# snt-arg/visual_sgraphs

Hardware: AMD Instinct MI355X
Metric: frames/sec ORB extract+match @640x480, 1000 feats; bit-exact vs CPU (higher is better)
Workload: dtype u8; 1 GPU; C2: 640x480 gray, nFeatures=1000, 8 levels, scale 1.2, FAST 20/7, extract + brute-force Hamming best2 match vs previous frame; parallelism=frame-sharded x1

## Files before the change

include/vsg_orb.h:

```cpp
#ifndef VSG_ORB_H
#define VSG_ORB_H

#include <stddef.h>
#include <stdint.h>

#ifdef __cplusplus
extern "C" {
#endif

#define VSG_OK 0
#define VSG_ERR_EMPTY_IMAGE (-1)
#define VSG_ERR_CAPACITY (-2)
#define VSG_ERR_UNSUPPORTED (-3)
#define VSG_ERR_NO_DEVICE (-4)
#define VSG_ERR_HIP (-5)
#define VSG_ERR_INVALID (-6)
#define VSG_ERR_BUSY (-7)

typedef struct vsg_keypoint {
  float x, y, size, angle, response;
  int32_t octave, class_id;
} vsg_keypoint;

typedef struct vsg_orb vsg_orb;

const char *vsg_last_error(void);
int vsg_device_count(void);


int vsg_orb_create(int nfeatures, float scale_factor, int nlevels, int ini_th_fast, int min_th_fast, int device,
                   int max_batch, vsg_orb **out);
void vsg_orb_destroy(vsg_orb *h);

int vsg_orb_get_tables(const vsg_orb *h, float *scale, float *inv_scale, float *sigma2, float *inv_sigma2,
                       int *features_per_level, int *umax16);

int vsg_orb_set_blur_taps(vsg_orb *h, const uint16_t taps[7]);

int vsg_orb_set_pyramid_tiling(vsg_orb *h, int which);

int vsg_orb_capacity(vsg_orb *h, int rows, int cols);

int vsg_orb_extract(vsg_orb *h, const uint8_t *gray, int rows, int cols, int stride, int lap0, int lap1,
                    vsg_keypoint *kps, uint8_t *desc, int capacity, int *n);

int vsg_orb_extract_batch(vsg_orb *h, const uint8_t *gray, int nframes, size_t frame_stride, int rows, int cols,
                          int stride, int lap0, int lap1, vsg_keypoint *kps, uint8_t *desc, int capacity, int *n,
                          int *mono_index);

int vsg_orb_extract_batch_device(vsg_orb *h, const uint8_t *d_gray, int nframes, size_t frame_stride, int rows,
                                 int cols, int stride, int lap0, int lap1, vsg_keypoint *d_kps, uint8_t *d_desc,
                                 int *d_counts, int capacity, void *stream);

int vsg_orb_set_gray_coeffs(vsg_orb *h, const int coeffs[3], int shift);
// ... 292 lines not shown
```

include/vsg_orb_debug.h:

```cpp
#ifndef VSG_ORB_DEBUG_H
#define VSG_ORB_DEBUG_H
#include "vsg_orb.h"

#ifdef __cplusplus
extern "C" {
#endif

int vsg_debug_device_sort(int device, uint64_t *items, int n);

int vsg_debug_call_profile(float us[4]);

enum {
  VSG_OCT_BLUR_MEMBATCH = 1,
  VSG_OCT_BLUR_MEMBATCH_FUSED = 2,
  VSG_OCT_FEW_MEMBATCH = 3,
  VSG_OCT_FEW_MEMBATCH_FUSED = 4,
  VSG_OCT_STANDALONE = 5
};

typedef struct vsg_launch_forms {
  int latency_chain;
  int pyramid_tiling;
  int fast_cells_per_wg;
  int fast_tile_pitch;
  int cand_segmented;
  int fused_blur;
  int octree_kernel;
  int octree_hist_big;
  int octree_label_bytes;
  int octree_lead;
  int self_slots;
  int orient_mirror;
  int cus;
  int total_cells;
  int nframes;
} vsg_launch_forms;

int vsg_debug_last_launch_forms(vsg_orb *h, vsg_launch_forms *out);

#ifdef __cplusplus
}
#endif
#endif
```

visual_sgraphs_amd/csrc/vsg_kernels.h:

```cpp
#pragma once
#include <hip/hip_runtime.h>

#include "vsg_common.h"
#include "vsg_geometry.h"

namespace vsg {
struct OutMirror {
  KeyPointPOD *kps = nullptr;
  uint8_t *desc = nullptr;
  int *counts = nullptr;
  int capacity = 0;
};
void launch_stereo(hipStream_t s, const PyrView &pl, const PyrView &pr, float mb, float mbf, const float *scale,
                   const float *invScale, int nlevels, const KeyPointPOD *kpsL, const uint8_t *descL, int nL,
                   const KeyPointPOD *kpsR, const uint8_t *descR, int nR, float *uRight, float *depth, int *sadBest);
void launch_cvt_gray(hipStream_t s, const uint8_t *src, size_t sframe, int spitch, int channels, int rgb_order, int rows,
                     int cols, uint8_t *dst, size_t dframe, int dpitch, const int coeffs[3], int shift, int nframes);
void launch_zero(hipStream_t s, int *p, int n);
void launch_ingest(hipStream_t s, const uint8_t *src, size_t sframe, int spitch, uint8_t *dst, size_t dframe, int dpitch,
                   int rows, int cols, int nframes);
void launch_export(hipStream_t s, const KeyPointPOD *kps, const uint8_t *desc, const int *counts, int src_cap,
                   void *h_kps, void *h_desc, int *h_counts, int dst_cap, int nframes);
void launch_resize(hipStream_t s, uint8_t *pyr, const FrameGeom *d_fg, const Short4 *d_tab, const Src0 &s0,
                   const FrameGeom &fg, int level, int nframes);
void launch_pyramid(hipStream_t s, uint8_t *pyr, const FrameGeom *d_fg, const Short4 *d_tile_tab, const Src0 &s0,
                    const PyrTile *d_tiles, int ntiles, int ldsA, int ldsB, int tabMax, int nframes, int *cand_count);
struct FastForm {
  int cells_per_wg = 0, tile_pitch = 0;
};
struct OctreeForm {
  int kernel = 0;
  int hist_big = 0, label_bytes = 0, lead = 0;
};
FastForm launch_fast(hipStream_t s, const uint8_t *pyr, const FrameGeom *d_fg, const FastCellRec *d_recs, const Src0 &s0,
                     uint32_t *cand, int *cand_count, int *cell_count, const FrameGeom &fg, int maxVh, int maxVw, int maxArea,
                     int nframes, int cus);
OctreeForm launch_octree(hipStream_t s, const FrameGeom *d_fg, const uint32_t *cand, const int *cand_count,
                         const CellDesc *d_cells, const int *cell_count, uint32_t *cand2, uint16_t *node_of, uint32_t *sel,
                         int *sel_count, const FrameGeom &fg, int maxQuota, int maxCellsPerLevel, int nframes,
                         const uint8_t *blur_pyr = nullptr, uint8_t *blur_out = nullptr, const Src0 *blur_s0 = nullptr);
size_t octree_lds_bytes(const FrameGeom &fg, int maxQuota, int maxCellsPerLevel);
constexpr int kOctBlurWaves = 4;
void launch_debug_sort(hipStream_t s, uint64_t *d_items, int n);
void launch_blur(hipStream_t s, const uint8_t *pyr, uint8_t *blur, const FrameGeom *d_fg, const Src0 &s0,
                 const FrameGeom &fg, int nframes);
void launch_slots(hipStream_t s, const FrameGeom *d_fg, const uint32_t *sel, const int *sel_count, int *flags,
                  int4 *slots, FrameHeader *hdr, int lap0, int lap1, int nframes);
void launch_orient_desc(hipStream_t s, const uint8_t *pyr, const uint8_t *blur, const FrameGeom *d_fg, const Src0 &s0,
                        const uint32_t *sel, const int *sel_count, const int4 *slots, const FrameHeader *hdr,
                        const int8_t *pattern, KeyPointPOD *kps, uint8_t *desc, int *counts, int capacity,
                        const FrameGeom &fg, int nframes, const OutMirror &mir, bool self_slots);
void launch_border_copy(hipStream_t s, const uint8_t *img, int w, int h, int pitch, uint8_t *dst, int dpitch, int b);
}
```

visual_sgraphs_amd/csrc/vsg_kernels.hip:

```cpp
#include <hip/hip_runtime.h>
#include <stdint.h>
#include <stdlib.h>

#include "vsg_common.h"
#include "vsg_ctx.h"
#include "vsg_geometry.h"
#include "vsg_math.h"
#include "vsg_octree_core.h"
#include "vsg_kernels.h"
#include "../../include/vsg_orb_debug.h"

namespace vsg {

__device__ __forceinline__ const uint8_t *level_ptr(const FrameGeom *fg, const Src0 &s0, const uint8_t *pyr, int frame,
                                                    int level, int &pitch) {
  if (level == 0) {
    pitch = s0.pitch;
    return s0.base + (size_t)frame * s0.frame_stride;
  }
  pitch = fg->lv[level].pitch;
  return pyr + (size_t)frame * fg->pyr_frame_bytes + fg->lv[level].img_off;
}

struct BlockXY {
// ... 982 lines not shown
        const int cutA = K < nA ? (int)posA[K] : 0x7FFFFFFF, cutB = K >= 1 ? (int)posB[K - 1] : e;
        const int cut = cutA < cutB ? cutA : cutB;
        __threadfence_block();
        if (lane == 0) stk[3 * sp] = lo, stk[3 * sp + 1] = cut, stk[3 * sp + 2] = depth;
        sp++;
        lo = cut;
      }
      if (sp == 0) break;
      --sp;
      __threadfence_block();
      lo = stk[3 * sp], hi = stk[3 * sp + 1], depth = stk[3 * sp + 2];
    }
  }
};

constexpr int kOctRegPts = 8;

constexpr int kOctThreads = 256;
constexpr int kOctWaves = 5;

struct SegSrc {
  const uint32_t *level_cand;
  const int *prefix;
  const int *segoff;
  int ncells;
  __device__ int cell_of(int p) const {
    int lo = 0, hi = ncells;
    while (hi - lo > 1) {
      const int mid = (lo + hi) >> 1;
      if (prefix[mid] <= p) lo = mid; else hi = mid;
// ... 48 lines not shown

constexpr int kOctFewFrames = 8;
struct OctArgs {
  const FrameGeom *fg;
  const uint32_t *cand;
  const int *cand_count;
  const CellDesc *cells;
  const int *cell_count;
  uint32_t *cand2;
  uint16_t *node_of;
  uint32_t *sel;
  int *sel_count;
  int cap, prefix_off;
  int lab_off, lab_cap;
  int hist_big;
};

template <int kMemU>
__device__ __forceinline__ void octree_block(const OctArgs &a, int level, int frame, uint8_t *oct_lds, int *wtot,
                                             int *sort_stack) {
  const FrameGeom *__restrict__ fg = a.fg;
  const uint32_t *__restrict__ cand = a.cand;
  const int *__restrict__ cand_count = a.cand_count;
  const CellDesc *__restrict__ cells = a.cells;
  const int *__restrict__ cell_count = a.cell_count;
  uint32_t *__restrict__ cand2 = a.cand2;
  uint16_t *__restrict__ node_of = a.node_of;
  uint32_t *__restrict__ sel = a.sel;
  int *__restrict__ sel_count = a.sel_count;
  const int cap = a.cap, prefix_off = a.prefix_off;
// ... 66 lines not shown
      __syncthreads();
      if (npts <= a.lab_cap)
        n = octree::distribute<kMemU>(g, P, list, npts, (uint16_t *)(oct_lds + a.lab_off), W, out);
      else
        n = octree::distribute<kMemU>(g, P, list, npts, node_of + coff, W, out);
    }
  } else {
    int npts = cand_count[frame * kMaxLevels + level];
    if (npts > L.cand_cap) npts = L.cand_cap;
    n = npts <= kOctRegPts * kOctThreads ? octree::distribute_reg<kOctRegPts>(g, P, cand + coff, npts, W, out)
                                         : octree::distribute<kMemU>(g, P, cand + coff, npts, node_of + coff, W, out);
  }
  if (threadIdx.x == 0) sel_count[frame * kMaxLevels + level] = n;
}

constexpr int kOctMemBatch = 8, kOctMemBatchFused = 1;

__global__ __launch_bounds__(kOctThreads) __attribute__((amdgpu_waves_per_eu(kOctWaves, kOctWaves))) void k_octree(OctArgs a) {
  extern __shared__ __attribute__((aligned(16))) uint8_t oct_lds[];
  __shared__ int wtot[2 * kMaxWaves];
  __shared__ int sort_stack[kSortStackInts];
  octree_block<kOctMemBatch>(a, blockIdx.x, blockIdx.y, oct_lds, wtot, sort_stack);
}
template <int kMemU>
__global__ __launch_bounds__(kOctThreads) __attribute__((amdgpu_waves_per_eu(4, 4))) void k_octree_few(OctArgs a) {
  extern __shared__ __attribute__((aligned(16))) uint8_t oct_lds[];
  __shared__ int wtot[2 * kMaxWaves];
  __shared__ int sort_stack[kSortStackInts];
  octree_block<kMemU>(a, blockIdx.x, blockIdx.y, oct_lds, wtot, sort_stack);
}

__global__ __launch_bounds__(256) void k_debug_sort(uint64_t *items, int n) {
  extern __shared__ __attribute__((aligned(16))) uint8_t dbg_lds[];
  __shared__ int wtot[2 * kMaxWaves];
  __shared__ int sort_stack[kSortStackInts];
  introsort::item_t *buf = (introsort::item_t *)dbg_lds;
  uint16_t *posA = (uint16_t *)(buf + n), *posB = posA + n + 2;
  BlockGroup g;
  g.tid = threadIdx.x;
  g.nthreads = blockDim.x;
  g.wtot = wtot;
  g.stk = sort_stack;
  for (int i = g.tid; i < n; i += g.nthreads) buf[i] = items[i];
  __syncthreads();
// ... 163 lines not shown
        u32x4 line;
        line.x = q_hi ? r02 : c0, line.y = q_hi ? r13 : c1, line.z = q_hi ? c2 : r20, line.w = q_hi ? c3 : r31;
        *(u32x4 *)(dst + (uint32_t)(o >> 2) * tile_row_bytes) = line;
      }
    }
  }
}

__global__ __launch_bounds__(256) void k_blur(const uint8_t *__restrict__ pyr, uint8_t *__restrict__ blur,
                                              const FrameGeom *__restrict__ fg, Src0 s0) {
  blur_block<kBlurAheadAlone>(pyr, blur, fg, s0, frame_major_block());
}

template <int kMemU>
__device__ __forceinline__ void octree_blur_body(const OctArgs &a, const uint8_t *__restrict__ pyr, uint8_t *__restrict__ blur,
                                                 const Src0 &s0, int nlevels, int nframes, int lead, uint8_t *oct_lds, int *wtot,
                                                 int *sort_stack) {
  static_assert(kOctThreads == 256, "the blur body is written for 256-thread workgroups");
  BlockXY blk = frame_major_block();
  if (lead > 0) {
    if (blk.x >= nlevels) blk.y -= lead;
    if (blk.y < 0 || blk.y >= nframes) return;
  }
  if (blk.x < nlevels)
    octree_block<kMemU>(a, blk.x, blk.y, oct_lds, wtot, sort_stack);
  else
    blur_block<kBlurAheadFused>(pyr, blur, a.fg, s0, BlockXY{blk.x - nlevels, blk.y});
}
template <int kMemU>
__global__ __launch_bounds__(kOctThreads) __attribute__((amdgpu_waves_per_eu(kOctBlurWaves, kOctBlurWaves))) void k_octree_blur(
    OctArgs a, const uint8_t *__restrict__ pyr, uint8_t *__restrict__ blur, Src0 s0, int nlevels, int nframes, int lead) {
  extern __shared__ __attribute__((aligned(16))) uint8_t oct_lds[];
  __shared__ int wtot[2 * kMaxWaves];
  __shared__ int sort_stack[kSortStackInts];
  octree_blur_body<kMemU>(a, pyr, blur, s0, nlevels, nframes, lead, oct_lds, wtot, sort_stack);
}

__device__ __forceinline__ void slots_of_frame(const FrameGeom *__restrict__ fg, const uint32_t *__restrict__ sel,
                                               const int *__restrict__ sel_count, int *__restrict__ flags,
                                               int4 *__restrict__ slots, FrameHeader *__restrict__ hdr, int lap0, int lap1,
                                               int frame, int *wtot, int *lstart) {
  const int tid = threadIdx.x;
  if (tid == 0) {
    int s = 0;
    for (int l = 0; l < fg->nlevels; l++) {
      lstart[l] = s;
      s += min(sel_count[frame * kMaxLevels + l], fg->lv[l].sel_cap);
    }
    for (int l = fg->nlevels; l <= kMaxLevels; l++) lstart[l] = s;
  }
// ... 566 lines not shown
    return launch_fast_t<kFastThreads, 52, 52, 2 * (128 / kFastThreads)>(s, pyr, d_fg, d_recs, s0, cand, cand_count, cell_count, fg, maxVh, maxArea, nframes, cus);
  else if (maxVw <= 56)
    return launch_fast_t<kFastThreads, 68, 68, 3 * (128 / kFastThreads)>(s, pyr, d_fg, d_recs, s0, cand, cand_count, cell_count, fg, maxVh, maxArea, nframes, cus);
  else
    return launch_fast_t<kFastThreads, 84, 84, 4 * (128 / kFastThreads)>(s, pyr, d_fg, d_recs, s0, cand, cand_count, cell_count, fg, maxVh, maxArea, nframes, cus);
}
size_t octree_lds_bytes(const FrameGeom &fg, int maxQuota, int maxCellsPerLevel) {
  const int cap = octree::node_capacity(maxQuota);
  const size_t prefix_off = (octree::work_bytes(cap, false) + 15) & ~(size_t)15;
  return prefix_off + (fg.cand_segmented ? (2 * (size_t)maxCellsPerLevel + 1) * 4 : 0);
}

OctreeForm launch_octree(hipStream_t s, const FrameGeom *d_fg, const uint32_t *cand, const int *cand_count,
                         const CellDesc *d_cells, const int *cell_count, uint32_t *cand2, uint16_t *node_of, uint32_t *sel,
                         int *sel_count, const FrameGeom &fg, int maxQuota, int maxCellsPerLevel, int nframes,
                         const uint8_t *blur_pyr, uint8_t *blur_out, const Src0 *blur_s0) {
  const int cap = octree::node_capacity(maxQuota);
  const size_t prefix_bytes = fg.cand_segmented ? (2 * (size_t)maxCellsPerLevel + 1) * 4 : 0;
  const size_t share = 36 * 1024;
  const bool hist_big = ((octree::work_bytes(cap, true) + 15) & ~(size_t)15) + prefix_bytes <= share;
  const int prefix_off = (int)((octree::work_bytes(cap, hist_big) + 15) & ~(size_t)15);
  const size_t work_lds = (size_t)prefix_off + prefix_bytes;
  const size_t lab_off = (work_lds + 15) & ~(size_t)15;
  const size_t lab_bytes = work_lds <= 64 * 1024 && lab_off + 4096 <= share ? share - lab_off : 0;
  const size_t lds = lab_bytes ? lab_off + lab_bytes : work_lds;
  int dev = 0;
  hipGetDevice(&dev);
  const OctArgs a = {d_fg, cand, cand_count, d_cells, cell_count, cand2, node_of, sel, sel_count, cap, prefix_off,
                     (int)lab_off, (int)(lab_bytes / 2), hist_big ? 1 : 0};
  const bool few = nframes <= kOctFewFrames;
  OctreeForm form;
  form.hist_big = hist_big ? 1 : 0, form.label_bytes = (int)lab_bytes;
  if (blur_out) {
    constexpr int kLead = 64;
    const int lead = nframes >= 4 * kLead ? kLead : 0;
    form.lead = lead;
    const dim3 grid(fg.nlevels + fg.total_blur_blocks, nframes + lead);
    if (few && 5 * work_lds > 160 * 1024) {
      lds_limit_ensure(5, dev, (const void *)k_octree_blur<kOctMemBatch>, lds);
      hipLaunchKernelGGL(k_octree_blur<kOctMemBatch>, grid, dim3(kOctThreads), lds, s, a, blur_pyr, blur_out, *blur_s0,
                         fg.nlevels, nframes, lead);
      form.kernel = VSG_OCT_BLUR_MEMBATCH;
    } else {
      lds_limit_ensure(2, dev, (const void *)k_octree_blur<kOctMemBatchFused>, lds);
      hipLaunchKernelGGL(k_octree_blur<kOctMemBatchFused>, grid, dim3(kOctThreads), lds, s, a, blur_pyr, blur_out, *blur_s0,
                         fg.nlevels, nframes, lead);
      form.kernel = VSG_OCT_BLUR_MEMBATCH_FUSED;
    }
    return form;
  }
  dim3 grid(fg.nlevels, nframes), block(kOctThreads);
  if (few) {
    lds_limit_ensure(6, dev, (const void *)k_octree_few<kOctMemBatch>, lds);
    hipLaunchKernelGGL(k_octree_few<kOctMemBatch>, grid, block, lds, s, a);
    form.kernel = VSG_OCT_FEW_MEMBATCH;
    return form;
  }
  if (5 * work_lds <= 160 * 1024) {
    lds_limit_ensure(4, dev, (const void *)k_octree_few<kOctMemBatchFused>, lds);
    hipLaunchKernelGGL(k_octree_few<kOctMemBatchFused>, grid, block, lds, s, a);
    form.kernel = VSG_OCT_FEW_MEMBATCH_FUSED;
    return form;
  }
  lds_limit_ensure(1, dev, (const void *)k_octree, lds);
  hipLaunchKernelGGL(k_octree, grid, block, lds, s, a);
  form.kernel = VSG_OCT_STANDALONE;
// ... 39 lines not shown
```

visual_sgraphs_amd/csrc/vsg_orb.hip:

```cpp
#include <hip/hip_runtime.h>

#include <cstdio>
#include <cstdlib>
#include <algorithm>
#include <atomic>
#include <condition_variable>
#include <mutex>
#include <thread>
#include <chrono>
#include <cmath>
#include <cstring>
#include <map>
#include <string>
#include <utility>
#include <vector>

#include "../../include/vsg_orb.h"
#include "../../include/vsg_orb_debug.h"
#include "vsg_common.h"
#include "vsg_ctx.h"
#include "vsg_frame_int.h"
#include "vsg_geometry.h"
#include "vsg_kernels.h"

// ... 109 lines not shown
  int rows = 0, cols = 0;
  uint16_t taps[7] = {18, 34, 49, 55, 49, 34, 18};
  int gray_coeffs[3] = {4899, 9617, 1868};
  int gray_shift = 14;
  int last_frames = 0;
  vsg_launch_forms forms = {};
  bool have_forms = false;
  FrameGeom *d_fg = nullptr;
  Short4 *d_tab = nullptr;
  CellDesc *d_cells = nullptr;
  FastCellRec *d_fast = nullptr;
  int *d_cell_count = nullptr;
  uint32_t *d_cand2 = nullptr;
  int pyr_tiling = 0;
  int force_tiling = -1;
  vsg_post_chain_fn post_fn = nullptr;
  void *post_ctx = nullptr;
  int cus = 256;
  PyrTile *d_ptiles[kPyrTilings] = {};
  Short4 *d_ptab[kPyrTilings] = {};
  uint8_t *d_in = nullptr;
  int in_pitch = 0;
  Slot slot[kSlots];
  int next_ticket = 0;
  hipStream_t s_h2d = nullptr, s_d2h = nullptr;
  const KeyPointPOD *last_kps = nullptr;
  const uint8_t *last_desc = nullptr;
  const int *last_counts = nullptr;
  int last_cap = 0;
  hipEvent_t ev_last = nullptr;
// ... 151 lines not shown
    HIP_TRY(hipMalloc(&h->d_ptab[i], sizeof(Short4) * (PT.tab.size() + 1)));
    if (!PT.tab.empty())
      HIP_TRY(hipMemcpy(h->d_ptab[i], PT.tab.data(), sizeof(Short4) * PT.tab.size(), hipMemcpyHostToDevice));
  }
  HIP_TRY(hipMalloc(&h->d_pyr, B * fg.pyr_frame_bytes));
  HIP_TRY(hipMalloc(&h->d_blur, B * fg.blur_frame_bytes));
  HIP_TRY(hipMemset(h->d_pyr, 0, B * fg.pyr_frame_bytes));
  HIP_TRY(hipMemset(h->d_blur, 0, B * fg.blur_frame_bytes));
  HIP_TRY(hipMalloc(&h->d_cand, B * fg.cand_frame * sizeof(uint32_t)));
  HIP_TRY(hipMalloc(&h->d_cand2, B * fg.cand_frame * sizeof(uint32_t)));
  HIP_TRY(hipMalloc(&h->d_cell_count, B * fg.total_cells * sizeof(int)));
  HIP_TRY(hipMemset(h->d_cell_count, 0, B * fg.total_cells * sizeof(int)));
  HIP_TRY(hipStreamSynchronize(nullptr));
  HIP_TRY(hipMalloc(&h->d_nodeof, B * fg.cand_frame * sizeof(uint16_t)));
  HIP_TRY(hipMalloc(&h->d_sel, B * fg.sel_frame * sizeof(uint32_t)));
  HIP_TRY(hipMalloc(&h->d_counts2, 2 * B * kMaxLevels * sizeof(int)));
  HIP_TRY(hipMalloc(&h->d_flags, B * fg.out_cap * sizeof(int)));
  HIP_TRY(hipMalloc(&h->d_slots, B * fg.out_cap * sizeof(int4)));
  HIP_TRY(hipMalloc(&h->d_hdr, B * sizeof(FrameHeader)));
  h->in_pitch = (cols + 3) & ~3;
  HIP_TRY(hipMalloc(&h->d_in, B * (size_t)rows * h->in_pitch + 64));
  h->rows = rows;
  h->cols = cols;
  rc = ensure_slot(h, 0);
  if (rc != VSG_OK) return rc;
  h->pyr_tiling = 0;
  {
    const PyrTiling &P0 = h->G.pyr[0], &P1 = h->G.pyr[1];
    const int nf = h->max_batch;
    if (fg.nlevels > 1 && P0.ok && P1.ok && P0.lds_bytes() <= kPyrLdsLimit && P1.lds_bytes() <= 50 * 1024 &&
        (long long)P1.tiles.size() * nf >= 2048) {
// ... 39 lines not shown

static int enqueue_pipeline(vsg_orb *h, const Src0 &s0, int nf, int lap0, int lap1, KeyPointPOD *d_kps,
                            uint8_t *d_desc, int *d_counts, int capacity, hipStream_t s) {
  h->last_src0 = s0;
  const FrameGeom &fg = h->G.fg;
  const bool tm = h->timing;
  const bool tmf = !tm && h->timing_fast;
  if (tm || tmf) harvest_timing(h);
  hipStream_t sb = h->serialize ? s : kOwnBlurStream;
  uint8_t *pyr = h->d_pyr, *blur = h->d_blur;
  uint32_t *cand = h->d_cand, *sel = h->d_sel;
  uint16_t *nodeof = h->d_nodeof;
  int *cell_count = h->d_cell_count;
  int *cand_count = h->d_counts2;
  int *sel_count = h->d_counts2 + (size_t)h->max_batch * kMaxLevels;
  int *flags = h->d_flags;
  int4 *slots = h->d_slots;
  FrameHeader *hdr = h->d_hdr;
  vsg_launch_forms &rec = h->forms;
  rec = vsg_launch_forms();
  rec.cus = h->cus, rec.total_cells = fg.total_cells, rec.nframes = nf, rec.cand_segmented = fg.cand_segmented ? 1 : 0;
  h->have_forms = true;
  Range r_all("vsg_orb: enqueue stage chain");
  if (tm) HIP_TRY(hipEventRecord(h->ev[0], s));
  int ti = -1;
  if (fg.nlevels > 1) {
    const PyrTiling &P0 = h->G.pyr[0], &P1 = h->G.pyr[1];
    const PyrTiling &PS = h->G.pyr[kPyrTilingSmall];
    const int forced = h->force_tiling;
    if (forced == 3)
// ... 21 lines not shown
  if (tm) HIP_TRY(hipEventRecord(h->ev[1], s));
  if (tm || tmf) HIP_TRY(hipEventRecord(h->ev[8], s));
  const FastForm ff = launch_fast(s, pyr, h->d_fg, h->d_fast, s0, cand, cand_count, cell_count, fg, h->G.fastMaxVh,
                                  h->G.fastMaxVw, h->G.fastMaxArea, nf, h->cus);
  rec.fast_cells_per_wg = ff.cells_per_wg, rec.fast_tile_pitch = ff.tile_pitch;
  if (tm || tmf) HIP_TRY(hipEventRecord(h->ev[2], s));
  constexpr int kFusedLdsWorkgroups = 5;
  const bool lds_fits = kFusedLdsWorkgroups * octree_lds_bytes(fg, h->G.maxQuota, h->G.maxCellsPerLevel) <= 160 * 1024;
  const bool fused_blur = !tm && sb != s && (lds_fits || (h->one_stream && nf <= 8));
  const bool self_slots = !tm && (lap1 < kEdgeThreshold || lap0 > lap1);
  rec.fused_blur = fused_blur ? 1 : 0, rec.self_slots = self_slots ? 1 : 0;
  OctreeForm of;
  if (fused_blur) {
    Range r_tail("DistributeOctTree (+ blur workgroups) + slots + IC_Angle / rBRIEF");
    of = launch_octree(s, h->d_fg, cand, cand_count, h->d_cells, cell_count, h->d_cand2, nodeof, sel, sel_count, fg,
                       h->G.maxQuota, h->G.maxCellsPerLevel, nf, pyr, blur, &s0);
    if (!self_slots) launch_slots(s, h->d_fg, sel, sel_count, flags, slots, hdr, lap0, lap1, nf);
  } else {
    HIP_TRY(hipEventRecord(h->ev_pyr, s));
    if (sb == kOwnBlurStream) {
      const int rs = need_stream(h, &h->s_blur);
      if (rs != VSG_OK) return rs;
      sb = h->s_blur;
    }
    const bool octree_first = sb != s;
    if (octree_first) {
      if (tm) HIP_TRY(hipEventRecord(h->ev[10], s));
      of = launch_octree(s, h->d_fg, cand, cand_count, h->d_cells, cell_count, h->d_cand2, nodeof, sel, sel_count, fg,
                         h->G.maxQuota, h->G.maxCellsPerLevel, nf);
      if (tm) HIP_TRY(hipEventRecord(h->ev[3], s));
    }
    HIP_TRY(hipStreamWaitEvent(sb, h->ev_pyr, 0));
    if (tm) HIP_TRY(hipEventRecord(h->ev[6], sb));
    launch_blur(sb, pyr, blur, h->d_fg, s0, fg, nf);
    if (tm) HIP_TRY(hipEventRecord(h->ev[7], sb));
    HIP_TRY(hipEventRecord(h->ev_blur, sb));
    Range r_tail("DistributeOctTree + slots + IC_Angle / rBRIEF");
    if (!octree_first) {
      if (tm) HIP_TRY(hipEventRecord(h->ev[10], s));
      of = launch_octree(s, h->d_fg, cand, cand_count, h->d_cells, cell_count, h->d_cand2, nodeof, sel, sel_count, fg,
                         h->G.maxQuota, h->G.maxCellsPerLevel, nf);
      if (tm) HIP_TRY(hipEventRecord(h->ev[3], s));
    }
    if (!self_slots) launch_slots(s, h->d_fg, sel, sel_count, flags, slots, hdr, lap0, lap1, nf);
    if (tm) HIP_TRY(hipEventRecord(h->ev[4], s));
    HIP_TRY(hipStreamWaitEvent(s, h->ev_blur, 0));
    if (tm) HIP_TRY(hipEventRecord(h->ev[9], s));
  }
  rec.octree_kernel = of.kernel, rec.octree_hist_big = of.hist_big, rec.octree_label_bytes = of.label_bytes;
  rec.octree_lead = of.lead;
  rec.orient_mirror = h->mirror.kps ? 1 : 0;
  launch_orient_desc(s, pyr, blur, h->d_fg, s0, sel, sel_count, slots, hdr, h->d_pattern, d_kps, d_desc, d_counts,
                     capacity, fg, nf, h->mirror, self_slots);
  if (tm) HIP_TRY(hipEventRecord(h->ev[5], s));
  if (tm || tmf) h->ev_pending = true;
  HIP_TRY(hipGetLastError());
  h->last_frames = nf;
  h->last_kps = d_kps, h->last_desc = d_desc, h->last_counts = d_counts, h->last_cap = capacity;
  HIP_TRY(hipEventRecord(h->ev_last, s));
  h->have_last = true;
  return VSG_OK;
}

static int wait_last(vsg_orb *h) {
  if (h->have_last) HIP_TRY(hipEventSynchronize(h->ev_last));
// ... 232 lines not shown
  if (tsum > 257) return VSG_ERR_UNSUPPORTED;
  memcpy(h->taps, taps, sizeof(h->taps));
  if (h->rows) {
    for (int k = 0; k < 7; k++) h->G.fg.taps[k] = taps[k];
    HIP_TRY(hipSetDevice(h->device));
    int rc = quiesce(h);
    if (rc != VSG_OK) return rc;
    HIP_TRY(hipMemcpy(h->d_fg, &h->G.fg, sizeof(FrameGeom), hipMemcpyHostToDevice));
  }
  return VSG_OK;
}

int vsg_orb_set_pyramid_tiling(vsg_orb *h, int which) {
  if (!h || which < -1 || which > kPyrTilings) return VSG_ERR_INVALID;
  h->force_tiling = which;
  return VSG_OK;
}

int vsg_orb_capacity(vsg_orb *h, int rows, int cols) {
  if (!h) return VSG_ERR_INVALID;
  if (rows <= 0 || cols <= 0) return VSG_ERR_EMPTY_IMAGE;
  int rc = ensure_geometry(h, rows, cols);
  if (rc != VSG_OK) return rc;
  return h->G.fg.out_cap;
}

int vsg_orb_extract_batch_device(vsg_orb *h, const uint8_t *d_gray, int nframes, size_t frame_stride, int rows,
                                 int cols, int stride, int lap0, int lap1, vsg_keypoint *d_kps, uint8_t *d_desc,
                                 int *d_counts, int capacity, void *stream) {
  if (!h || !d_kps || !d_desc || !d_counts || nframes < 1 || nframes > h->max_batch) return VSG_ERR_INVALID;
// ... 679 lines not shown
  launch_debug_sort(c->stream, (uint64_t *)c->d_buf, n);
  HIP_TRY(hipGetLastError());
  HIP_TRY(hipMemcpyAsync(c->h_pin, c->d_buf, sizeof(uint64_t) * n, hipMemcpyDeviceToHost, c->stream));
  HIP_TRY(hipStreamSynchronize(c->stream));
  memcpy(items, c->h_pin, sizeof(uint64_t) * n);
  return VSG_OK;
}

int vsg_debug_last_launch_forms(vsg_orb *h, vsg_launch_forms *out) {
  if (!h || !out) return VSG_ERR_INVALID;
  if (!h->have_forms) {
    set_err("vsg_debug_last_launch_forms: the handle has not enqueued a batch yet");
    return VSG_ERR_INVALID;
  }
  *out = h->forms;
  return VSG_OK;
}

int vsg_orb_get_timing(vsg_orb *h, float *ms_out, int cap) {
  if (!h) return VSG_ERR_INVALID;
  harvest_timing(h);
  for (int i = 0; i < kStages && i < cap; i++) ms_out[i] = h->acc_n ? (float)(h->acc_ms[i] / h->acc_n) : 0.f;
  return kStages;
}

}
```

visual_sgraphs_amd/orb.py:

```python
import ctypes as C
from pathlib import Path

import numpy as np

import os

_PKG = Path(__file__).resolve().parent
LIB_PATH = Path(os.environ["VSG_LIB"]) if os.environ.get("VSG_LIB") else _PKG / "libvsg_orb.so"

KP_DTYPE = np.dtype([("x", "<f4"), ("y", "<f4"), ("size", "<f4"), ("angle", "<f4"), ("response", "<f4"),
                     ("octave", "<i4"), ("class_id", "<i4")])
assert KP_DTYPE.itemsize == 28

VSG_OK = 0
ERRORS = {-1: "VSG_ERR_EMPTY_IMAGE", -2: "VSG_ERR_CAPACITY", -3: "VSG_ERR_UNSUPPORTED", -4: "VSG_ERR_NO_DEVICE",
          -5: "VSG_ERR_HIP", -6: "VSG_ERR_INVALID", -7: "VSG_ERR_BUSY"}

_u8p = C.POINTER(C.c_uint8)
_i32p = C.POINTER(C.c_int32)
_u32p = C.POINTER(C.c_uint32)
_f32p = C.POINTER(C.c_float)
_u16p = C.POINTER(C.c_uint16)

EXPORTS = [
# ... 9 lines not shown
    "vsg_vocab_info", "vsg_bow_transform", "vsg_distinctive_descriptors", "vsg_debug_device_sort",
    "vsg_search_for_triangulation", "vsg_search_by_bow_kf_f_stereo",
    "vsg_thread_release", "vsg_thread_arena_growths", "vsg_debug_call_profile", "vsg_orb_time_stats", "vsg_host_register", "vsg_host_unregister", "vsg_host_alloc", "vsg_host_free", "vsg_orb_slots",
    "vsg_orb_submit_batch", "vsg_orb_wait", "vsg_orb_copy_pyramid", "vsg_frame_create", "vsg_frame_destroy",
    "vsg_frame_upload", "vsg_frame_from_extractor", "vsg_frame_size", "vsg_frame_copy_grid",
    "vsg_frame_features_in_area", "vsg_frame_search_by_projection", "vsg_frame_search_by_projection_last",
    "vsg_frame_search_by_projection_sim3", "vsg_frame_search_by_projection_kf", "vsg_frame_search_by_sim3",
    "vsg_frame_fuse", "vsg_frame_fuse_sim3", "vsg_fuse_decide", "vsg_frame_search_for_initialization",
    "vsg_frame_search_by_bow_kf_f", "vsg_frame_search_by_bow_kf_kf", "vsg_frame_bow_transform", "vsg_frame_stereo_bow_search",
    "vsg_frame_search_for_triangulation",
    "vsg_frame_stereo_matches",
    "vsg_shard_last_error", "vsg_shard_record_bytes", "vsg_shard_record_desc_offset", "vsg_shard_frame_owner",
    "vsg_shard_stream_owner", "vsg_shard_unique_id", "vsg_shard_create", "vsg_shard_destroy", "vsg_shard_all_gather",
    "vsg_shard_record", "vsg_shard_world", "vsg_shard_send_recv_boundary", "vsg_shard_boundary_record",
    "vsg_copy_d2d_async",
    "vsg_orb_set_pyramid_tiling", "vsg_shard_rank", "vsg_camera_image_bounds", "vsg_frame_from_extractor_undistort",
    "vsg_orb_extract_to_frame",
    "vsg_orb_extract_to_frame_rgbd", "vsg_depth_map_scale", "vsg_rgbd_depth_batch_device",
    "vsg_host_kind", "vsg_orb_set_direct_registered",
    "vsg_vocab_score", "vsg_kfdb_create", "vsg_kfdb_destroy", "vsg_kfdb_add", "vsg_kfdb_erase", "vsg_kfdb_clear",
    "vsg_kfdb_clear_map", "vsg_kfdb_set_map", "vsg_kfdb_set_covisibility", "vsg_kfdb_detect_relocalization_candidates",
    "vsg_kfdb_detect_n_best_candidates",
    "vsg_mappoints_create", "vsg_mappoints_destroy", "vsg_mappoints_capacity", "vsg_mappoints_update",
    "vsg_mappoints_read", "vsg_frame_is_in_frustum", "vsg_frame_search_local_points",
    "vsg_debug_last_launch_forms",
]

LAUNCH_FORM_FIELDS = ("latency_chain", "pyramid_tiling", "fast_cells_per_wg", "fast_tile_pitch", "cand_segmented",
                      "fused_blur", "octree_kernel", "octree_hist_big", "octree_label_bytes", "octree_lead", "self_slots",
                      "orient_mirror", "cus", "total_cells", "nframes")
OCT_BLUR_MEMBATCH, OCT_BLUR_MEMBATCH_FUSED, OCT_FEW_MEMBATCH, OCT_FEW_MEMBATCH_FUSED, OCT_STANDALONE = 1, 2, 3, 4, 5


class _LaunchForms(C.Structure):
    _fields_ = [(n, C.c_int) for n in LAUNCH_FORM_FIELDS]


class FramePose(C.Structure):
    _fields_ = [("Rcw", C.c_float * 9), ("tcw", C.c_float * 3), ("Ow", C.c_float * 3), ("fx", C.c_float),
                ("fy", C.c_float), ("cx", C.c_float), ("cy", C.c_float), ("mbf", C.c_float),
                ("log_scale_factor", C.c_float), ("n_levels", C.c_int32)]

    @classmethod
    def make(cls, Rcw, tcw, Ow, fx, fy, cx, cy, mbf, log_scale_factor, n_levels):
        p = cls()
# ... 56 lines not shown
    if _lib is not None:
        return _lib
    if not LIB_PATH.exists():
        raise RuntimeError(f"{LIB_PATH} is missing: run `python -m visual_sgraphs_amd.build` "
                           "(the ORB front-end has no CPU fallback)")
    _share_torch_hip_runtime()
    L = C.CDLL(str(LIB_PATH))
    L.vsg_last_error.restype = C.c_char_p
    L.vsg_orb_create.argtypes = [C.c_int, C.c_float, C.c_int, C.c_int, C.c_int, C.c_int, C.c_int, C.POINTER(C.c_void_p)]
    L.vsg_orb_destroy.argtypes = [C.c_void_p]
    L.vsg_orb_destroy.restype = None
    L.vsg_orb_get_tables.argtypes = [C.c_void_p, _f32p, _f32p, _f32p, _f32p, _i32p, _i32p]
    L.vsg_orb_set_blur_taps.argtypes = [C.c_void_p, _u16p]
    L.vsg_orb_capacity.argtypes = [C.c_void_p, C.c_int, C.c_int]
    L.vsg_orb_set_pyramid_tiling.argtypes = [C.c_void_p, C.c_int]
    L.vsg_orb_extract.argtypes = [C.c_void_p, _u8p, C.c_int, C.c_int, C.c_int, C.c_int, C.c_int, C.c_void_p, _u8p,
                                  C.c_int, _i32p]
    L.vsg_orb_extract_batch.argtypes = [C.c_void_p, _u8p, C.c_int, C.c_size_t, C.c_int, C.c_int, C.c_int, C.c_int,
                                        C.c_int, C.c_void_p, _u8p, C.c_int, _i32p, _i32p]
    L.vsg_orb_extract_batch_device.argtypes = [C.c_void_p, C.c_void_p, C.c_int, C.c_size_t, C.c_int, C.c_int, C.c_int,
                                               C.c_int, C.c_int, C.c_void_p, C.c_void_p, C.c_void_p, C.c_int,
                                               C.c_void_p]
    L.vsg_orb_level_size.argtypes = [C.c_void_p, C.c_int, _i32p, _i32p]
    L.vsg_orb_copy_pyramid_level.argtypes = [C.c_void_p, C.c_int, C.c_int, C.c_int, _u8p, C.c_int]
    L.vsg_orb_copy_blurred_level.argtypes = [C.c_void_p, C.c_int, C.c_int, _u8p, C.c_int]
    L.vsg_orb_copy_candidates.argtypes = [C.c_void_p, C.c_int, C.c_int, _u32p, C.c_int]
    L.vsg_orb_copy_selected.argtypes = [C.c_void_p, C.c_int, C.c_int, _u32p, C.c_int]
    L.vsg_orb_enable_timing.argtypes = [C.c_void_p, C.c_int]
    L.vsg_orb_get_timing.argtypes = [C.c_void_p, _f32p, C.c_int]
    L.vsg_orb_set_serialize.argtypes = [C.c_void_p, C.c_int]
# ... 229 lines not shown

    def features_per_level(self):
        return self._tables()[4]

    def umax(self):
        return self._tables()[5]

    def set_blur_taps(self, taps):
        t = np.ascontiguousarray(taps, dtype=np.uint16)
        assert t.shape == (7,)
        _check(self._L.vsg_orb_set_blur_taps(self._h, _p(t, _u16p)), "vsg_orb_set_blur_taps")

    def set_pyramid_tiling(self, which):
        _check(self._L.vsg_orb_set_pyramid_tiling(self._h, int(which)), "vsg_orb_set_pyramid_tiling")

    def set_direct_registered(self, on=True):
        _check(self._L.vsg_orb_set_direct_registered(self._h, int(on)), "vsg_orb_set_direct_registered")

    def capacity(self, rows, cols):
        return _check(self._L.vsg_orb_capacity(self._h, int(rows), int(cols)), "vsg_orb_capacity")

    def __call__(self, image, mask=None, vLappingArea=(0, 0)):
        if image is None or image.size == 0:
            return -1, np.zeros(0, KP_DTYPE), np.zeros((0, 32), np.uint8)
        img = np.asarray(image)
        assert img.dtype == np.uint8 and img.ndim == 2, "CV_8UC1 expected (ORBextractor.cc:1091)"
        if img.strides[1] != 1:
            img = np.ascontiguousarray(img)
        rows, cols = img.shape
        cap = self.capacity(rows, cols)
# ... 1043 lines not shown
```

Before: 388,500 frames/s.

## Pack small coarse pyramid levels' octree distribution into one wave per level

Adds a wavefront-level octree distribution path, so the coarsest pyramid levels (up to four) each run on a single 64-lane wave. Four such levels share one 256-thread workgroup, each with its own LDS slice and scan stack, which cuts the number of octree workgroups per frame. If a level has too many points or needs more LDS than its slice, the workgroup falls back to the full block path, and a per-level flag records which path ran. The aim is to stop spending whole workgroups on tiny levels. The cost is more LDS per block, which may lower occupancy, plus extra branching.

```diff
diff --git a/include/vsg_orb.h b/include/vsg_orb.h
--- a/include/vsg_orb.h
+++ b/include/vsg_orb.h
@@ -38,6 +38,8 @@
 int vsg_orb_set_blur_taps(vsg_orb *h, const uint16_t taps[7]);
 
 int vsg_orb_set_pyramid_tiling(vsg_orb *h, int which);
+
+int vsg_orb_set_octree_wave_levels(vsg_orb *h, int levels);
 
 int vsg_orb_capacity(vsg_orb *h, int rows, int cols);
 
diff --git a/include/vsg_orb_debug.h b/include/vsg_orb_debug.h
--- a/include/vsg_orb_debug.h
+++ b/include/vsg_orb_debug.h
@@ -34,6 +34,8 @@
   int cus;
   int total_cells;
   int nframes;
+  int octree_wave_levels;
+  int octree_wave_fallbacks;
 } vsg_launch_forms;
 
 int vsg_debug_last_launch_forms(vsg_orb *h, vsg_launch_forms *out);
diff --git a/visual_sgraphs_amd/csrc/vsg_kernels.h b/visual_sgraphs_amd/csrc/vsg_kernels.h
--- a/visual_sgraphs_amd/csrc/vsg_kernels.h
+++ b/visual_sgraphs_amd/csrc/vsg_kernels.h
@@ -31,6 +31,7 @@
 struct OctreeForm {
   int kernel = 0;
   int hist_big = 0, label_bytes = 0, lead = 0;
+  int wave_levels = 0;
 };
 FastForm launch_fast(hipStream_t s, const uint8_t *pyr, const FrameGeom *d_fg, const FastCellRec *d_recs, const Src0 &s0,
                      uint32_t *cand, int *cand_count, int *cell_count, const FrameGeom &fg, int maxVh, int maxVw, int maxArea,
@@ -38,7 +39,7 @@
 OctreeForm launch_octree(hipStream_t s, const FrameGeom *d_fg, const uint32_t *cand, const int *cand_count,
                          const CellDesc *d_cells, const int *cell_count, uint32_t *cand2, uint16_t *node_of, uint32_t *sel,
                          int *sel_count, const FrameGeom &fg, int maxQuota, int maxCellsPerLevel, int nframes,
-                         const uint8_t *blur_pyr = nullptr, uint8_t *blur_out = nullptr, const Src0 *blur_s0 = nullptr);
+                         int wave_levels, int *wave_form, const uint8_t *blur_pyr = nullptr, uint8_t *blur_out = nullptr, const Src0 *blur_s0 = nullptr);
 size_t octree_lds_bytes(const FrameGeom &fg, int maxQuota, int maxCellsPerLevel);
 constexpr int kOctBlurWaves = 4;
 void launch_debug_sort(hipStream_t s, uint64_t *d_items, int n);
diff --git a/visual_sgraphs_amd/csrc/vsg_kernels.hip b/visual_sgraphs_amd/csrc/vsg_kernels.hip
--- a/visual_sgraphs_amd/csrc/vsg_kernels.hip
+++ b/visual_sgraphs_amd/csrc/vsg_kernels.hip
@@ -1020,6 +1020,50 @@
   }
 };
 
+struct WaveGroup : BlockGroup {
+  __device__ void sync() {
+    __threadfence_block();
+    __builtin_amdgcn_wave_barrier();
+  }
+  __device__ int exclusive_scan(int *a, int n) {
+    const int per = (n + 63) >> 6;
+    const int lo = min(tid * per, n), hi = min(lo + per, n);
+    int s = 0;
+    for (int i = lo; i < hi; i++) s += a[i];
+    const int incl = wave_inclusive_scan(s);
+    int run = incl - s;
+    for (int i = lo; i < hi; i++) {
+      const int v = a[i];
+      a[i] = run;
+      run += v;
+    }
+    sync();
+    return __builtin_amdgcn_readlane(incl, 63);
+  }
+  __device__ int exclusive_scan2(int *a, int *b, int n, int *total_b) {
+    const int per = (n + 63) >> 6;
+    const int lo = min(tid * per, n), hi = min(lo + per, n);
+    int sa = 0, sb = 0;
+    for (int i = lo; i < hi; i++) sa += a[i], sb += b[i];
+    const int ia = wave_inclusive_scan(sa), ib = wave_inclusive_scan(sb);
+    int ra = ia - sa, rb = ib - sb;
+    for (int i = lo; i < hi; i++) {
+      const int va = a[i], vb = b[i];
+      a[i] = ra, b[i] = rb;
+      ra += va, rb += vb;
+    }
+    sync();
+    *total_b = __builtin_amdgcn_readlane(ib, 63);
+    return __builtin_amdgcn_readlane(ia, 63);
+  }
+  __device__ int exclusive_scan2_one(int a, int b, int *ex_a, int *ex_b, int *total_b) {
+    const int ia = wave_inclusive_scan(a), ib = wave_inclusive_scan(b);
+    *ex_a = ia - a, *ex_b = ib - b;
+    *total_b = __builtin_amdgcn_readlane(ib, 63);
+    return __builtin_amdgcn_readlane(ia, 63);
+  }
+};
+
 constexpr int kOctRegPts = 8;
 
 constexpr int kOctThreads = 256;
@@ -1098,6 +1142,8 @@
   int cap, prefix_off;
   int lab_off, lab_cap;
   int hist_big;
+  int wave_levels, wave_slice;
+  int *wave_form;
 };
 
 template <int kMemU>
@@ -1194,20 +1240,106 @@
   if (threadIdx.x == 0) sel_count[frame * kMaxLevels + level] = n;
 }
 
+constexpr int kOctWaveGroup = kOctThreads / 64;
+constexpr int kWaveStackInts = 64;
+static_assert(kOctWaveGroup * kWaveStackInts + kOctWaveGroup <= kSortStackInts, "the waves' range stacks and fallback flags share sort_stack");
+__host__ __device__ inline size_t octree_wave_prefix_off(int quota) {
+  return (octree::work_bytes(octree::node_capacity(quota), false) + 15) & ~(size_t)15;
+}
+__device__ __forceinline__ bool octree_wave(const OctArgs &a, int level, int frame, uint8_t *lds, int *stk) {
+  const FrameGeom *__restrict__ fg = a.fg;
+  const LevelGeom &L = fg->lv[level];
+  const int cap = octree::node_capacity(L.quota), ncells = L.nCols * L.nRows;
+  const size_t prefix_off = octree_wave_prefix_off(L.quota);
+  if (cap >= 1024 || prefix_off + (fg->cand_segmented ? (2 * (size_t)ncells + 1) * 4 : 0) > (size_t)a.wave_slice) return false;
+  octree::Params P;
+  P.N = L.quota;
+  P.height = L.oct_height;
+  P.nIni = L.nIni;
+  P.iniUL = L.iniUL;
+  P.iniThresh = L.iniThresh;
+  P.nCols = L.nCols;
+  P.wCell = L.wCell;
+  P.hCell = L.hCell;
+  octree::Work W;
+  octree::carve(W, lds, cap, false);
+  WaveGroup g;
+  g.tid = threadIdx.x & 63;
+  g.nthreads = 64;
+  g.wtot = nullptr;
+  g.stk = stk;
+  const size_t coff = (size_t)frame * fg->cand_frame + L.cand_off;
+  uint32_t *out = a.sel + (size_t)frame * fg->sel_frame + L.sel_off;
+  int n;
+  if (fg->cand_segmented) {
+    int *prefix = (int *)(lds + prefix_off), *segoff = prefix + ncells + 1;
+    const int *cc = a.cell_count + (size_t)frame * fg->total_cells + L.cell_base;
+    for (int i = g.tid; i < ncells; i += 64) {
+      prefix[i] = cc[i];
+      segoff[i] = a.cells[L.cell_base + i].cand_off;
+    }
+    g.sync();
+    const int npts = g.exclusive_scan(prefix, ncells);
+    if (npts > kOctRegPts * 64) return false;
+    if (g.tid == 0) prefix[ncells] = npts;
+    g.sync();
+    SegRegPts<kOctRegPts> pts;
+    pts.src = SegSrc{a.cand + coff, prefix, segoff, ncells};
+    n = octree::distribute_pts(g, P, pts, npts, W, out);
+  } else {
+    int npts = a.cand_count[frame * kMaxLevels + level];
+    if (npts > L.cand_cap) npts = L.cand_cap;
+    if (npts > kOctRegPts * 64) return false;
+    n = octree::distribute_reg<kOctRegPts>(g, P, a.cand + coff, npts, W, out);
+  }
+  if (g.tid == 0) a.sel_count[frame * kMaxLevels + level] = n;
+  return true;
+}
+
+__host__ __device__ inline int octree_blocks_per_frame(int nlevels, int wave_levels) {
+  return nlevels - wave_levels + (wave_levels + kOctWaveGroup - 1) / kOctWaveGroup;
+}
+template <int kMemU>
+__device__ __forceinline__ void octree_levels(const OctArgs &a, int x, int frame, uint8_t *oct_lds, int *wtot, int *sort_stack) {
+  const int nlevels = a.fg->nlevels, nbig = nlevels - a.wave_levels;
+  int level0 = x, todo = 1;
+  if (x >= nbig) {
+    level0 = nbig + (x - nbig) * kOctWaveGroup;
+    const int nlv = min(kOctWaveGroup, nlevels - level0), wave = threadIdx.x >> 6;
+    int *fell = sort_stack + kOctWaveGroup * kWaveStackInts;
+    if (wave < nlv) {
+      const bool ok = octree_wave(a, level0 + wave, frame, oct_lds + (size_t)wave * a.wave_slice, sort_stack + wave * kWaveStackInts);
+      if ((threadIdx.x & 63) == 0) {
+        fell[wave] = ok ? 0 : 1;
+        a.wave_form[frame * kMaxLevels + level0 + wave] = ok ? 1 : 0;
+      }
+    }
+    __syncthreads();
+    todo = 0;
+    for (int w = 0; w < nlv; w++) todo |= fell[w] << w;
+    if (todo == 0) return;
+    __syncthreads();
+  }
+  for (int w = 0; todo >> w; w++)
+    if ((todo >> w) & 1) {
+      octree_block<kMemU>(a, level0 + w, frame, oct_lds, wtot, sort_stack);
+    }
+}
+
 constexpr int kOctMemBatch = 8, kOctMemBatchFused = 1;
 
 __global__ __launch_bounds__(kOctThreads) __attribute__((amdgpu_waves_per_eu(kOctWaves, kOctWaves))) void k_octree(OctArgs a) {
   extern __shared__ __attribute__((aligned(16))) uint8_t oct_lds[];
   __shared__ int wtot[2 * kMaxWaves];
   __shared__ int sort_stack[kSortStackInts];
-  octree_block<kOctMemBatch>(a, blockIdx.x, blockIdx.y, oct_lds, wtot, sort_stack);
+  octree_levels<kOctMemBatch>(a, blockIdx.x, blockIdx.y, oct_lds, wtot, sort_stack);
 }
 template <int kMemU>
 __global__ __launch_bounds__(kOctThreads) __attribute__((amdgpu_waves_per_eu(4, 4))) void k_octree_few(OctArgs a) {
   extern __shared__ __attribute__((aligned(16))) uint8_t oct_lds[];
   __shared__ int wtot[2 * kMaxWaves];
   __shared__ int sort_stack[kSortStackInts];
-  octree_block<kMemU>(a, blockIdx.x, blockIdx.y, oct_lds, wtot, sort_stack);
+  octree_levels<kMemU>(a, blockIdx.x, blockIdx.y, oct_lds, wtot, sort_stack);
 }
 
 __global__ __launch_bounds__(256) void k_debug_sort(uint64_t *items, int n) {
@@ -1401,26 +1533,26 @@
 
 template <int kMemU>
 __device__ __forceinline__ void octree_blur_body(const OctArgs &a, const uint8_t *__restrict__ pyr, uint8_t *__restrict__ blur,
-                                                 const Src0 &s0, int nlevels, int nframes, int lead, uint8_t *oct_lds, int *wtot,
+                                                 const Src0 &s0, int noct, int nframes, int lead, uint8_t *oct_lds, int *wtot,
                                                  int *sort_stack) {
   static_assert(kOctThreads == 256, "the blur body is written for 256-thread workgroups");
   BlockXY blk = frame_major_block();
   if (lead > 0) {
-    if (blk.x >= nlevels) blk.y -= lead;
+    if (blk.x >= noct) blk.y -= lead;
     if (blk.y < 0 || blk.y >= nframes) return;
   }
-  if (blk.x < nlevels)
-    octree_block<kMemU>(a, blk.x, blk.y, oct_lds, wtot, sort_stack);
+  if (blk.x < noct)
+    octree_levels<kMemU>(a, blk.x, blk.y, oct_lds, wtot, sort_stack);
   else
-    blur_block<kBlurAheadFused>(pyr, blur, a.fg, s0, BlockXY{blk.x - nlevels, blk.y});
+    blur_block<kBlurAheadFused>(pyr, blur, a.fg, s0, BlockXY{blk.x - noct, blk.y});
 }
 template <int kMemU>
 __global__ __launch_bounds__(kOctThreads) __attribute__((amdgpu_waves_per_eu(kOctBlurWaves, kOctBlurWaves))) void k_octree_blur(
-    OctArgs a, const uint8_t *__restrict__ pyr, uint8_t *__restrict__ blur, Src0 s0, int nlevels, int nframes, int lead) {
+    OctArgs a, const uint8_t *__restrict__ pyr, uint8_t *__restrict__ blur, Src0 s0, int noct, int nframes, int lead) {
   extern __shared__ __attribute__((aligned(16))) uint8_t oct_lds[];
   __shared__ int wtot[2 * kMaxWaves];
   __shared__ int sort_stack[kSortStackInts];
-  octree_blur_body<kMemU>(a, pyr, blur, s0, nlevels, nframes, lead, oct_lds, wtot, sort_stack);
+  octree_blur_body<kMemU>(a, pyr, blur, s0, noct, nframes, lead, oct_lds, wtot, sort_stack);
 }
 
 __device__ __forceinline__ void slots_of_frame(const FrameGeom *__restrict__ fg, const uint32_t *__restrict__ sel,
@@ -2017,7 +2149,7 @@
 OctreeForm launch_octree(hipStream_t s, const FrameGeom *d_fg, const uint32_t *cand, const int *cand_count,
                          const CellDesc *d_cells, const int *cell_count, uint32_t *cand2, uint16_t *node_of, uint32_t *sel,
                          int *sel_count, const FrameGeom &fg, int maxQuota, int maxCellsPerLevel, int nframes,
-                         const uint8_t *blur_pyr, uint8_t *blur_out, const Src0 *blur_s0) {
+                         int wave_levels, int *wave_form, const uint8_t *blur_pyr, uint8_t *blur_out, const Src0 *blur_s0) {
   const int cap = octree::node_capacity(maxQuota);
   const size_t prefix_bytes = fg.cand_segmented ? (2 * (size_t)maxCellsPerLevel + 1) * 4 : 0;
   const size_t share = 36 * 1024;
@@ -2026,33 +2158,46 @@
   const size_t work_lds = (size_t)prefix_off + prefix_bytes;
   const size_t lab_off = (work_lds + 15) & ~(size_t)15;
   const size_t lab_bytes = work_lds <= 64 * 1024 && lab_off + 4096 <= share ? share - lab_off : 0;
-  const size_t lds = lab_bytes ? lab_off + lab_bytes : work_lds;
+  size_t lds = lab_bytes ? lab_off + lab_bytes : work_lds;
+  constexpr size_t kOctWaveSlice = 9472;
+  if (wave_levels != 0 && lds < kOctWaveGroup * kOctWaveSlice) lds = kOctWaveGroup * kOctWaveSlice;
   int dev = 0;
   hipGetDevice(&dev);
+  constexpr int kOctWaveLevels = 4;
+  const int wave_slice = (int)((lds / kOctWaveGroup) & ~(size_t)15);
+  int wl = wave_levels < fg.nlevels ? wave_levels : fg.nlevels;
+  if (wave_levels < 0) {
+    for (wl = 0; wl < kOctWaveLevels && wl < fg.nlevels / 2; wl++) {
+      const LevelGeom &L = fg.lv[fg.nlevels - 1 - wl];
+      const size_t need = octree_wave_prefix_off(L.quota) + (fg.cand_segmented ? (2 * (size_t)L.nCols * L.nRows + 1) * 4 : 0);
+      if (need > (size_t)wave_slice) break;
+    }
+  }
+  const int noct = octree_blocks_per_frame(fg.nlevels, wl);
   const OctArgs a = {d_fg, cand, cand_count, d_cells, cell_count, cand2, node_of, sel, sel_count, cap, prefix_off,
-                     (int)lab_off, (int)(lab_bytes / 2), hist_big ? 1 : 0};
+                     (int)lab_off, (int)(lab_bytes / 2), hist_big ? 1 : 0, wl, wave_slice, wave_form};
   const bool few = nframes <= kOctFewFrames;
   OctreeForm form;
-  form.hist_big = hist_big ? 1 : 0, form.label_bytes = (int)lab_bytes;
+  form.hist_big = hist_big ? 1 : 0, form.label_bytes = (int)lab_bytes, form.wave_levels = wl;
   if (blur_out) {
     constexpr int kLead = 64;
     const int lead = nframes >= 4 * kLead ? kLead : 0;
     form.lead = lead;
-    const dim3 grid(fg.nlevels + fg.total_blur_blocks, nframes + lead);
+    const dim3 grid(noct + fg.total_blur_blocks, nframes + lead);
     if (few && 5 * work_lds > 160 * 1024) {
       lds_limit_ensure(5, dev, (const void *)k_octree_blur<kOctMemBatch>, lds);
       hipLaunchKernelGGL(k_octree_blur<kOctMemBatch>, grid, dim3(kOctThreads), lds, s, a, blur_pyr, blur_out, *blur_s0,
-                         fg.nlevels, nframes, lead);
+                         noct, nframes, lead);
       form.kernel = VSG_OCT_BLUR_MEMBATCH;
     } else {
       lds_limit_ensure(2, dev, (const void *)k_octree_blur<kOctMemBatchFused>, lds);
       hipLaunchKernelGGL(k_octree_blur<kOctMemBatchFused>, grid, dim3(kOctThreads), lds, s, a, blur_pyr, blur_out, *blur_s0,
-                         fg.nlevels, nframes, lead);
+                         noct, nframes, lead);
       form.kernel = VSG_OCT_BLUR_MEMBATCH_FUSED;
     }
     return form;
   }
-  dim3 grid(fg.nlevels, nframes), block(kOctThreads);
+  dim3 grid(noct, nframes), block(kOctThreads);
   if (few) {
     lds_limit_ensure(6, dev, (const void *)k_octree_few<kOctMemBatch>, lds);
     hipLaunchKernelGGL(k_octree_few<kOctMemBatch>, grid, block, lds, s, a);
diff --git a/visual_sgraphs_amd/csrc/vsg_orb.hip b/visual_sgraphs_amd/csrc/vsg_orb.hip
--- a/visual_sgraphs_amd/csrc/vsg_orb.hip
+++ b/visual_sgraphs_amd/csrc/vsg_orb.hip
@@ -147,6 +147,7 @@
   uint32_t *d_cand2 = nullptr;
   int pyr_tiling = 0;
   int force_tiling = -1;
+  int wave_levels = -1;
   vsg_post_chain_fn post_fn = nullptr;
   void *post_ctx = nullptr;
   int cus = 256;
@@ -328,7 +329,7 @@
   HIP_TRY(hipStreamSynchronize(nullptr));
   HIP_TRY(hipMalloc(&h->d_nodeof, B * fg.cand_frame * sizeof(uint16_t)));
   HIP_TRY(hipMalloc(&h->d_sel, B * fg.sel_frame * sizeof(uint32_t)));
-  HIP_TRY(hipMalloc(&h->d_counts2, 2 * B * kMaxLevels * sizeof(int)));
+  HIP_TRY(hipMalloc(&h->d_counts2, 3 * B * kMaxLevels * sizeof(int)));
   HIP_TRY(hipMalloc(&h->d_flags, B * fg.out_cap * sizeof(int)));
   HIP_TRY(hipMalloc(&h->d_slots, B * fg.out_cap * sizeof(int4)));
   HIP_TRY(hipMalloc(&h->d_hdr, B * sizeof(FrameHeader)));
@@ -398,6 +399,7 @@
   int *cell_count = h->d_cell_count;
   int *cand_count = h->d_counts2;
   int *sel_count = h->d_counts2 + (size_t)h->max_batch * kMaxLevels;
+  int *wave_form = h->d_counts2 + 2 * (size_t)h->max_batch * kMaxLevels;
   int *flags = h->d_flags;
   int4 *slots = h->d_slots;
   FrameHeader *hdr = h->d_hdr;
@@ -449,7 +451,7 @@
   if (fused_blur) {
     Range r_tail("DistributeOctTree (+ blur workgroups) + slots + IC_Angle / rBRIEF");
     of = launch_octree(s, h->d_fg, cand, cand_count, h->d_cells, cell_count, h->d_cand2, nodeof, sel, sel_count, fg,
-                       h->G.maxQuota, h->G.maxCellsPerLevel, nf, pyr, blur, &s0);
+                       h->G.maxQuota, h->G.maxCellsPerLevel, nf, h->wave_levels, wave_form, pyr, blur, &s0);
     if (!self_slots) launch_slots(s, h->d_fg, sel, sel_count, flags, slots, hdr, lap0, lap1, nf);
   } else {
     HIP_TRY(hipEventRecord(h->ev_pyr, s));
@@ -462,7 +464,7 @@
     if (octree_first) {
       if (tm) HIP_TRY(hipEventRecord(h->ev[10], s));
       of = launch_octree(s, h->d_fg, cand, cand_count, h->d_cells, cell_count, h->d_cand2, nodeof, sel, sel_count, fg,
-                         h->G.maxQuota, h->G.maxCellsPerLevel, nf);
+                         h->G.maxQuota, h->G.maxCellsPerLevel, nf, h->wave_levels, wave_form);
       if (tm) HIP_TRY(hipEventRecord(h->ev[3], s));
     }
     HIP_TRY(hipStreamWaitEvent(sb, h->ev_pyr, 0));
@@ -474,7 +476,7 @@
     if (!octree_first) {
       if (tm) HIP_TRY(hipEventRecord(h->ev[10], s));
       of = launch_octree(s, h->d_fg, cand, cand_count, h->d_cells, cell_count, h->d_cand2, nodeof, sel, sel_count, fg,
-                         h->G.maxQuota, h->G.maxCellsPerLevel, nf);
+                         h->G.maxQuota, h->G.maxCellsPerLevel, nf, h->wave_levels, wave_form);
       if (tm) HIP_TRY(hipEventRecord(h->ev[3], s));
     }
     if (!self_slots) launch_slots(s, h->d_fg, sel, sel_count, flags, slots, hdr, lap0, lap1, nf);
@@ -483,7 +485,7 @@
     if (tm) HIP_TRY(hipEventRecord(h->ev[9], s));
   }
   rec.octree_kernel = of.kernel, rec.octree_hist_big = of.hist_big, rec.octree_label_bytes = of.label_bytes;
-  rec.octree_lead = of.lead;
+  rec.octree_lead = of.lead, rec.octree_wave_levels = of.wave_levels;
   rec.orient_mirror = h->mirror.kps ? 1 : 0;
   launch_orient_desc(s, pyr, blur, h->d_fg, s0, sel, sel_count, slots, hdr, h->d_pattern, d_kps, d_desc, d_counts,
                      capacity, fg, nf, h->mirror, self_slots);
@@ -746,6 +748,12 @@
 int vsg_orb_set_pyramid_tiling(vsg_orb *h, int which) {
   if (!h || which < -1 || which > kPyrTilings) return VSG_ERR_INVALID;
   h->force_tiling = which;
+  return VSG_OK;
+}
+
+int vsg_orb_set_octree_wave_levels(vsg_orb *h, int levels) {
+  if (!h || levels < -1 || levels > kMaxLevels) return VSG_ERR_INVALID;
+  h->wave_levels = levels;
   return VSG_OK;
 }
 
@@ -1455,6 +1463,17 @@
     return VSG_ERR_INVALID;
   }
   *out = h->forms;
+  out->octree_wave_fallbacks = 0;
+  const int wl = h->forms.octree_wave_levels, nf = h->forms.nframes, nl = h->G.fg.nlevels;
+  if (wl > 0 && nf > 0) {
+    int rc = wait_last(h);
+    if (rc != VSG_OK) return rc;
+    std::vector<int> flags((size_t)nf * kMaxLevels);
+    HIP_TRY(hipMemcpy(flags.data(), h->d_counts2 + 2 * (size_t)h->max_batch * kMaxLevels, flags.size() * sizeof(int),
+                      hipMemcpyDeviceToHost));
+    for (int f = 0; f < nf; f++)
+      for (int l = nl - wl; l < nl; l++) out->octree_wave_fallbacks += flags[(size_t)f * kMaxLevels + l] == 0;
+  }
   return VSG_OK;
 }
 
diff --git a/visual_sgraphs_amd/orb.py b/visual_sgraphs_amd/orb.py
--- a/visual_sgraphs_amd/orb.py
+++ b/visual_sgraphs_amd/orb.py
@@ -47,7 +47,7 @@
     "vsg_shard_stream_owner", "vsg_shard_unique_id", "vsg_shard_create", "vsg_shard_destroy", "vsg_shard_all_gather",
     "vsg_shard_record", "vsg_shard_world", "vsg_shard_send_recv_boundary", "vsg_shard_boundary_record",
     "vsg_copy_d2d_async",
-    "vsg_orb_set_pyramid_tiling", "vsg_shard_rank", "vsg_camera_image_bounds", "vsg_frame_from_extractor_undistort",
+    "vsg_orb_set_pyramid_tiling", "vsg_orb_set_octree_wave_levels", "vsg_shard_rank", "vsg_camera_image_bounds", "vsg_frame_from_extractor_undistort",
     "vsg_orb_extract_to_frame",
     "vsg_orb_extract_to_frame_rgbd", "vsg_depth_map_scale", "vsg_rgbd_depth_batch_device",
     "vsg_host_kind", "vsg_orb_set_direct_registered",
@@ -61,7 +61,7 @@
 
 LAUNCH_FORM_FIELDS = ("latency_chain", "pyramid_tiling", "fast_cells_per_wg", "fast_tile_pitch", "cand_segmented",
                       "fused_blur", "octree_kernel", "octree_hist_big", "octree_label_bytes", "octree_lead", "self_slots",
-                      "orient_mirror", "cus", "total_cells", "nframes")
+                      "orient_mirror", "cus", "total_cells", "nframes", "octree_wave_levels", "octree_wave_fallbacks")
 OCT_BLUR_MEMBATCH, OCT_BLUR_MEMBATCH_FUSED, OCT_FEW_MEMBATCH, OCT_FEW_MEMBATCH_FUSED, OCT_STANDALONE = 1, 2, 3, 4, 5
 
 
@@ -148,6 +148,7 @@
     L.vsg_orb_set_blur_taps.argtypes = [C.c_void_p, _u16p]
     L.vsg_orb_capacity.argtypes = [C.c_void_p, C.c_int, C.c_int]
     L.vsg_orb_set_pyramid_tiling.argtypes = [C.c_void_p, C.c_int]
+    L.vsg_orb_set_octree_wave_levels.argtypes = [C.c_void_p, C.c_int]
     L.vsg_orb_extract.argtypes = [C.c_void_p, _u8p, C.c_int, C.c_int, C.c_int, C.c_int, C.c_int, C.c_void_p, _u8p,
                                   C.c_int, _i32p]
     L.vsg_orb_extract_batch.argtypes = [C.c_void_p, _u8p, C.c_int, C.c_size_t, C.c_int, C.c_int, C.c_int, C.c_int,
@@ -407,6 +408,9 @@
     def set_pyramid_tiling(self, which):
         _check(self._L.vsg_orb_set_pyramid_tiling(self._h, int(which)), "vsg_orb_set_pyramid_tiling")
 
+    def set_octree_wave_levels(self, levels):
+        _check(self._L.vsg_orb_set_octree_wave_levels(self._h, int(levels)), "vsg_orb_set_octree_wave_levels")
+
     def set_direct_registered(self, on=True):
         _check(self._L.vsg_orb_set_direct_registered(self._h, int(on)), "vsg_orb_set_direct_registered")
 
```

Result: slower. 379,300 frames/s (-2.4%).
